# Total-RD/pymgrid

Measured on AMD Instinct MI355X. Metric: microgrid env-steps/sec, higher is better.
Workload: dtype f64

## Files before the change

pymgrid_amd/_lib.py:

```python
import ctypes as C
import json
import os
import re
import subprocess
import sys

_PKG = os.path.dirname(os.path.abspath(__file__))
_ROOT = os.path.dirname(_PKG)
LIB_PATH = os.environ.get("MGX_LIB") or os.path.join(_PKG, "libmgx.so")
SOURCES = [os.path.join(_PKG, "csrc", f) for f in ("mgx_abi.hip", "mgx_fused.hip", "mgx_kernels.hpp", "mgx_core.hpp", "mgx_episodes.hip",
                                                      "mgx_step_episodes.hip")] + \
          [os.path.join(_ROOT, "include", "mgx.h")]
FUSED_PARTS = 6
EPISODE_PARTS = 2
STEP_EPISODE_PARTS = 2

HIPCC_FLAGS = ["--offload-arch=gfx950", "-O3", "-std=c++17", "-ffp-contract=off", "-fno-fast-math", "-fPIC"]

MGX_OK, MGX_ERR_INVALID, MGX_ERR_UNSUPPORTED, MGX_ERR_RANGE, MGX_ERR_DEVICE = range(5)
V_GENSET_RANGE, V_BATTERY_LIMIT, V_GRID_LIMIT, V_GENSET_GOAL, V_GENSET_NEGATIVE, V_NEGATIVE_LIMIT = 1, 2, 4, 8, 16, 32
V_EXPAND_CONSUME, V_EXPAND_PRODUCE, V_EXPAND_SIGN = 64, 128, 256
V_EXPAND = V_EXPAND_CONSUME | V_EXPAND_PRODUCE | V_EXPAND_SIGN
V_ASSERTS = V_GENSET_GOAL | V_GENSET_NEGATIVE | V_NEGATIVE_LIMIT | V_EXPAND
ABI_VERSION = 9
ABI_MINOR = 3
TUNABLES = ("win_threads", "win_group", "win_pairs", "win_min_lds", "prefetch_pool", "multi_generic", "multi_small_own",
            "grid_major_copy", "fleet_byvalue", "launch_threads", "multi_static", "fleet_episodes")
MAX_INSTANCES = 8


class MgxError(RuntimeError):
    def __init__(self, code, message):
        super().__init__(f"[mgx error {code}] {message}")
        self.code = code


c_double_p = C.POINTER(C.c_double)
c_u32_p = C.POINTER(C.c_uint32)
c_u8_p = C.POINTER(C.c_uint8)
c_i32_p = C.POINTER(C.c_int32)


class Layout(C.Structure):
    _fields_ = [(n, C.c_int32) for n in (
# ... 321 lines not shown
```

pymgrid_amd/csrc/mgx_core.hpp:

```cpp
#pragma once

#include <hip/hip_runtime.h>
#include <stdint.h>

#include "../../include/mgx.h"

namespace mgx {

enum : int { F_GENSET = 1, F_BATTERY = 2, F_GRID = 4, F_GRID_FIRST = 8 };

enum LogCol : int {
    LC_REWARD = 0, LC_FIXED_PROVIDED, LC_FIXED_ABSORBED, LC_CTRL_PROVIDED, LC_CTRL_ABSORBED,
    LC_OVERALL_PROVIDED, LC_OVERALL_ABSORBED,
    LC_LOAD_MET, LC_RENEWABLE_USED, LC_CURTAILMENT, LC_LOSS_LOAD, LC_OVERGENERATION, LC_UNBALANCED_REWARD,
    LC_COMMON_END,
    LC_GENSET_N = 4, LC_BATTERY_N = 5, LC_GRID_N = 4
};

struct KArgs {
    mgx_columns c;
    int32_t N, T, H, final_step;
    int32_t obs_dim, log_dim;
    int32_t n_load, n_pv;
    int32_t n_genset, n_battery, n_grid;
    int32_t obs_f32;
    int32_t act_f32;
    int32_t obs_state_only;
    int32_t done_bits;
    int32_t obs_colpitch;
    int32_t col_load, col_pv, col_gen, col_bat, col_grid;
    int32_t shaper;
    int32_t noise_increase;
    uint64_t noise_seed;
    int32_t *t_dev;
    int32_t g0, g1;
    const int32_t *grid_final;
    int32_t row_mask;
    int32_t *ep_off, *ep_final;
// ... 40 lines not shown
        if (prev == gridDim.x - 1) {
            const int32_t t = __hip_atomic_load(&a.t_dev[0], __ATOMIC_RELAXED, __HIP_MEMORY_SCOPE_AGENT);
            __hip_atomic_store(&a.t_dev[2], 0, __ATOMIC_RELAXED, __HIP_MEMORY_SCOPE_AGENT);
            __hip_atomic_store(&a.t_dev[0], t + k, __ATOMIC_RELEASE, __HIP_MEMORY_SCOPE_AGENT);
        }
    }
}

__device__ __forceinline__ int32_t resolve_t_obs(const KArgs &a, int32_t t) { return a.t_dev ? a.t_dev[0] + t : t; }

__device__ __forceinline__ int32_t resolve_k(const KArgs &a, int32_t t0, int32_t K)
{
    if (a.t_dev && t0 + K > a.T) { a.t_dev[1] = 1; return a.T - t0; }
    return K;
}

struct Params {
    double bat_cmin, bat_cmax, bat_C, bat_D, bat_eta, bat_cost;
    double gen_rmin, gen_rmax, gen_cost, gen_co2, gen_cco2;
    uint32_t gen_times;
    double grid_imp, grid_exp, grid_cco2;
    double ll_cost, og_cost;
};

struct State {
    double charge, soc;
    uint32_t status;
};

struct Derived {
    double bat_lo, bat_sp;
    double gen_sp;
    double grid_lo, grid_sp;
};

struct Inputs {
    double a_goal, a_gen, a_bat, a_grid;
    double load, pv;
    double g_pimp, g_pexp, g_co2, g_stat;
};

struct Outputs {
    double reward;
    double fixed_provided, fixed_absorbed, ctrl_provided, ctrl_absorbed, overall_provided, overall_absorbed;
    double load_met, renewable_used, curtailment, loss_load, overgeneration, unbalanced_reward;
    double genset_production, genset_co2, genset_reward;
    double discharge_amount, charge_amount, battery_reward, soc_pre, charge_pre;
    double grid_import, grid_export, grid_co2, grid_reward;
    uint32_t violations;
};

__device__ __forceinline__ double space_spread(double lo, double hi)
{
    double s = hi - lo;
    return s == 0.0 ? 1.0 : s;
}
__device__ __forceinline__ double space_denorm(double lo, double hi, double v) { return lo + space_spread(lo, hi) * v; }
__device__ __forceinline__ double space_norm(double lo, double hi, double v) { return (v - lo) / space_spread(lo, hi); }

__device__ __forceinline__ double py_min(double a, double b)
{
    double r;
    asm("v_min_f64 %0, %1, %2" : "=v"(r) : "v"(a), "v"(b));
    return r;
}
__device__ __forceinline__ double py_max(double a, double b)
{
    double r;
    asm("v_max_f64 %0, %1, %2" : "=v"(r) : "v"(a), "v"(b));
    return r;
}
__device__ __forceinline__ double py_clip(double x, double lo, double hi) { return py_min(py_max(x, lo), hi); }

template <int F>
__device__ __forceinline__ void derive(const Params &p, Derived &d)
{
    if constexpr (F & F_BATTERY) {
        d.bat_lo = -p.bat_D / p.bat_eta;
        d.bat_sp = space_spread(d.bat_lo, p.bat_C * p.bat_eta);
    }
    if constexpr (F & F_GENSET) d.gen_sp = space_spread(0.0, p.gen_rmax);
    if constexpr (F & F_GRID) {
        d.grid_lo = -1 * p.grid_exp;
        d.grid_sp = space_spread(d.grid_lo, p.grid_imp);
    }
}

constexpr int PP = MGX_PROFILE_PITCH;

__host__ __device__ __forceinline__ bool factorised(const mgx_columns &c) { return c.base_load != nullptr; }

struct GridFactors {
    double lr, pr;
    uint32_t lp, pp, cp, pat;
};

template <int F>
__device__ __forceinline__ void load_factors(const mgx_columns &c, int64_t i, GridFactors &f)
{
    f.lr = c.load_ratio[i]; f.pr = c.pv_ratio[i];
    f.lp = c.load_profile[i]; f.pp = c.pv_profile[i];
    f.cp = 0u; f.pat = 0u;
    if constexpr (F & F_GRID) { f.cp = c.co2_profile[i]; f.pat = c.tariff[i]; }
}

__device__ __forceinline__ int64_t base_index(int32_t pm, int64_t row, uint32_t p)
{
    return pm ? (int64_t)p * pm + row : row * PP + p;
}

__device__ __forceinline__ double fact_load(double base, double ratio) { return -1.0 * fabs(base * ratio); }
__device__ __forceinline__ double fact_pv(double base, double ratio) { return fabs(base * ratio); }

__device__ __forceinline__ double tariff_price(int32_t pattern, int32_t row)
{
    const int32_t h = row % 24;
    if (pattern == 1) return (h >= 12 && h < 18) ? 0.59 : ((h < 8 || h >= 21) ? 0.22 : 0.29);
// ... 163 lines not shown
            }
            if (gs != cur) { if (gs == 0) down -= 1; else up -= 1; }
        }
    }
    return (uint32_t)cur | ((uint32_t)gs << 8) | ((uint32_t)(up & 0xff) << 16) | ((uint32_t)(down & 0xff) << 24);
}

__device__ __forceinline__ int genset_next_status(uint32_t st, int goal)
{
    const int cur = st & 0xff, up = (st >> 16) & 0xff, down = st >> 24;
    if (goal) return (cur || up == 0) ? 1 : 0;
    return (!cur || down == 0) ? 0 : 1;
}

template <int F>
__device__ __forceinline__ bool genset_wave_is_instant(const Params &p, const State &s)
{
    if constexpr (F & F_GENSET)
        return __all((p.gen_times == 0u) && (s.status == 0u || s.status == 0x0101u)) != 0;
    return false;
}

__device__ __forceinline__ double battery_max_production(const Params &p, double charge)
{
    const double b = charge - p.bat_cmin;
    return py_min(p.bat_D, b) * p.bat_eta;
}
__device__ __forceinline__ double battery_max_consumption(const Params &p, double charge)
{
    const double b = p.bat_cmax - charge;
    return py_min(p.bat_C, b) / p.bat_eta;
}

template <int F, bool HAVE_Q = false>
__device__ __forceinline__ void step_core(const Params &p, const Derived &d, State &s, const Inputs &in, bool normalized,
                                          bool want_soc, bool gen_instant, Outputs &o, double bat_q = 0.0)
{
    double prov = 0.0, absb = 0.0, reward = 0.0;
    uint32_t viol = 0u;

    const double L = -1 * in.load;
    o.load_met = L;
    absb += L; reward += 0.0;
    o.fixed_provided = prov; o.fixed_absorbed = absb;

    if constexpr (F & F_GENSET) {
        if (gen_instant) {
            const uint32_t g = in.a_goal > 0.5 ? 1u : 0u;
            s.status = g | (g << 8);
        } else {
            s.status = genset_update_status(s.status, p.gen_times, in.a_goal);
        }
        const double x = normalized ? 0.0 + d.gen_sp * in.a_gen : in.a_gen;
        const double cur = (double)(s.status & 0xff);
        const double mx = cur * p.gen_rmax, mn = cur * p.gen_rmin;
        const double e = py_clip(x, mn, mx);
        viol |= ((x > mx) || (x < mn) ? 1u : 0u) | (!(in.a_goal >= 0.0 && in.a_goal <= 1.0) ? 8u : 0u) | (x < 0.0 ? 16u : 0u);
        const double co2 = p.gen_co2 * e;
        const double cost = p.gen_cost * e + p.gen_cco2 * co2;
        o.genset_production = e; o.genset_co2 = co2; o.genset_reward = -1.0 * cost;
        prov += e; reward += o.genset_reward;
    }

    auto step_battery = [&]() __attribute__((always_inline)) {
        const double x = normalized ? d.bat_lo + d.bat_sp * in.a_bat : in.a_bat;
        o.soc_pre = s.soc; o.charge_pre = s.charge;
        const bool sink = x < 0;
        const double room = p.bat_cmax - s.charge;
        const double num_sink = py_min(p.bat_C, room);
        const double mp = battery_max_production(p, s.charge);
        const double e_src = py_clip(x, 0.0, mp);
        const double num = sink ? num_sink : -1.0 * e_src;
        double q;
        if constexpr (HAVE_Q) q = bat_q; else q = num / p.bat_eta;
        const double ex = -1.0 * x;
        const double e_sink = py_min(ex, q);
        const double e = sink ? e_sink : e_src;
        viol |= (sink ? (ex > q) : (x > mp)) ? 2u : 0u;
        viol |= !((sink ? e_sink : e_src) >= 0) ? 32u : 0u;
        const double internal = sink ? e * p.bat_eta : ((num < 0) ? q : num * p.bat_eta);
        o.charge_amount = sink ? e : 0.0;
        o.discharge_amount = sink ? 0.0 : e;
        absb += o.charge_amount; prov += o.discharge_amount;
        s.charge = py_max(s.charge + internal, p.bat_cmin);
        if (want_soc) s.soc = s.charge / p.bat_cmax;
        o.battery_reward = -1.0 * (fabs(internal) * p.bat_cost);
        reward += o.battery_reward;
    };
    auto step_grid = [&]() __attribute__((always_inline)) {
        const double x = normalized ? d.grid_lo + d.grid_sp * in.a_grid : in.a_grid;
        const bool sink = x < 0;
        const double ex = -1.0 * x, mc = p.grid_exp * in.g_stat;
        const double e_exp = py_min(ex, mc);
        const double mp = p.grid_imp * in.g_stat;
        const double e_imp = py_clip(x, 0.0, mp);
        viol |= (sink ? (ex > mc) : (x > mp)) ? 4u : 0u;
        viol |= !((sink ? e_exp : e_imp) >= 0) ? 32u : 0u;
        const double co2 = sink ? 0.0 : e_imp * in.g_co2;
        const double cco2 = -1.0 * p.grid_cco2 * co2;
        o.grid_export = sink ? e_exp : 0.0;
        o.grid_import = sink ? 0.0 : e_imp;
        o.grid_co2 = co2;
        o.grid_reward = sink ? in.g_pexp * e_exp + cco2 : -1 * in.g_pimp * e_imp + cco2;
        absb += o.grid_export; prov += o.grid_import;
        reward += o.grid_reward;
    };
    if constexpr ((F & F_GRID_FIRST) != 0) {
        if constexpr (F & F_GRID) step_grid();
        if constexpr (F & F_BATTERY) step_battery();
    } else {
        if constexpr (F & F_BATTERY) step_battery();
        if constexpr (F & F_GRID) step_grid();
    }

    const double difference = prov - absb;
    o.ctrl_provided = prov - o.fixed_provided;
    o.ctrl_absorbed = absb - o.fixed_absorbed;

    const bool excess = difference > 0;
    const double need = -difference;
    const double used = excess ? 0.0 : py_min(need, in.pv);
    o.renewable_used = used; o.curtailment = in.pv - used;
    const double loss = excess ? 0.0 : need - used;
    const double over = excess ? difference : 0.0;
    o.loss_load = loss; o.overgeneration = over;
    o.unbalanced_reward = -1.0 * (excess ? p.og_cost * over : p.ll_cost * loss);
    prov += used; reward += 0.0;
    prov += loss;
    absb += over;
    reward += o.unbalanced_reward;
    o.overall_provided = prov; o.overall_absorbed = absb;
    o.reward = reward;
    o.violations = viol;
}

struct PLWords {
    uint32_t w[12];
    int32_t n_actions;
};

__device__ __forceinline__ uint32_t pl_select(const PLWords &tab, int32_t id)
{
    uint32_t w = tab.w[0];
#pragma unroll
    for (int j = 1; j < 12; j++) w = (id == j && j < tab.n_actions) ? tab.w[j] : w;
    return w;
}

__device__ __forceinline__ bool pl_isclose0(double rem)
{
    return fabs(rem - 0.0) <= 1e-4 + 1e-5 * fabs(0.0);
}

__device__ __forceinline__ double pl_energy(double rem, double mn, double mx, double mc, bool is_sink)
{
    const double produce = py_clip(rem, mn, mx);
    const double consume = is_sink ? py_max(rem, -1.0 * mc) : 0.0;
    return pl_isclose0(rem) ? 0.0 : ((rem > 0) ? produce : consume);
}

template <int F, bool CHECK = false>
__device__ __forceinline__ void populate_core(const Params &p, const State &s, uint32_t word, Inputs &in, double &bat_q,
                                              double total_load, double renewable, bool gen_instant = false,
                                              uint32_t *xviol = nullptr, bool check_sign = true)
{
    const double rem0 = total_load - renewable;
    double g_mx[2] = {0.0, 0.0}, g_mn[2] = {0.0, 0.0};
    if constexpr (F & F_GENSET) {
#pragma unroll
        for (int act = 0; act < 2; act++) {
            const double ns = gen_instant ? (double)act : (double)genset_next_status(s.status, act);
            g_mx[act] = ns * p.gen_rmax; g_mn[act] = ns * p.gen_rmin;
        }
    }
    double r_mx = 0.0, r_mc = 0.0;
    if constexpr (F & F_GRID) { r_mx = p.grid_imp * in.g_stat; r_mc = p.grid_exp * in.g_stat; }

    constexpr int NSLOT = ((F & F_GENSET) != 0) + ((F & F_BATTERY) != 0) + ((F & F_GRID) != 0);
    constexpr int NS = NSLOT > 0 ? NSLOT : 1;
    uint32_t el[NS];
#pragma unroll
    for (int k = 0; k < NS; k++) el[k] = (k < NSLOT) ? (word >> (4 * k)) & 0xfu : 0u;
    auto cheap = [&](int mod, int act, double rem) -> double {
        double e = 0.0;
        if constexpr ((F & F_GENSET) && (F & F_GRID))
            e = (mod == 0) ? pl_energy(rem, g_mn[act], g_mx[act], 0.0, false) : pl_energy(rem, 0.0, r_mx, r_mc, true);
        else if constexpr (F & F_GENSET)
            e = pl_energy(rem, g_mn[act], g_mx[act], 0.0, false);
        else if constexpr (F & F_GRID)
            e = pl_energy(rem, 0.0, r_mx, r_mc, true);
        return e;
    };

    double remB = rem0;
    if constexpr (F & F_BATTERY) {
        double rem = rem0;
        bool seen = false;
#pragma unroll
        for (int k = 0; k < NSLOT - 1; k++) {
            const bool valid = (el[k] & 8u) != 0;
            const int mod = el[k] & 3u, act = (el[k] >> 2) & 1u;
            const bool isB = valid && mod == 1;
            seen = seen || isB;
            rem -= (valid && !seen) ? cheap(mod, act, rem) : 0.0;
            remB = seen ? remB : rem;
        }
    }
    double eB = 0.0;
    bat_q = 0.0;
    if constexpr (F & F_BATTERY) {
        const bool close = pl_isclose0(remB);
        const bool produce = !close && remB > 0;
        const double mp = battery_max_production(p, s.charge);
        const double room = p.bat_cmax - s.charge;
        const double num_sink = py_min(p.bat_C, room);
        const double e_src = py_clip(remB, 0.0, mp);
        const double num = (close || produce) ? -1.0 * (produce ? e_src : 0.0) : num_sink;
        const double q = num / p.bat_eta;
        const double e_snk = py_max(remB, -1.0 * q);
        eB = close ? 0.0 : (produce ? e_src : e_snk);
        bat_q = q;
    }
    double rem = rem0, c_goal = 0.0, c_gen = 0.0, c_grid = 0.0;
    uint32_t xv = 0u;
    if constexpr (CHECK) xv = (check_sign && !(total_load >= 0 && renewable >= 0)) ? 256u : 0u;
#pragma unroll
    for (int k = 0; k < NSLOT; k++) {
        const bool valid = (el[k] & 8u) != 0;
        const int mod = el[k] & 3u, act = (el[k] >> 2) & 1u;
        const double e = (mod == 1) ? eB : cheap(mod, act, rem);
        if constexpr (CHECK) {
            const bool close = pl_isclose0(rem), produce = !close && rem > 0, consume = !close && !produce;
            const double mc = (mod == 1) ? bat_q : r_mc;
            uint32_t bad = (produce && !(e >= 0)) ? 128u : 0u;
            bad = (consume && !(rem <= 0.0)) ? 256u : bad;
            bad = (consume && rem <= 0.0 && mod != 0 && !(mc >= 0)) ? 64u : bad;
            xv = (xv == 0u && valid) ? bad : xv;
        }
        const bool isG = valid && mod == 0, isR = valid && mod == 2;
        c_goal = isG ? (double)act : c_goal;
        c_gen = isG ? e : c_gen;
        c_grid = isR ? e : c_grid;
        rem -= valid ? e : 0.0;
    }
    in.a_goal = c_goal; in.a_gen = c_gen; in.a_bat = eB; in.a_grid = c_grid;
    if constexpr (CHECK) { if (xviol) *xviol = xv; }
}

template <int F>
__device__ __forceinline__ double shaped_reward(int32_t shaper, const Outputs &o)
{
// ... 1054 lines not shown
```

pymgrid_amd/csrc/mgx_episodes.hip:

```cpp
#include "mgx_kernels.hpp"

#ifndef MGX_EPISODE_PART
#error "compile with -DMGX_EPISODE_PART=<0..MGX_EPISODE_PARTS-1>"
#endif

#if MGX_EPISODE_PART == 0
#define MGX_PART_FLAGS(X) X(0) X(1) X(2) X(3) X(4) X(5)
#elif MGX_EPISODE_PART == 1
#define MGX_PART_FLAGS(X) X(6) X(7) X(14) X(15)
#else
#error "MGX_EPISODE_PART out of range"
#endif

#define MGX_CAT2(a, b) a##b
#define MGX_CAT(a, b) MGX_CAT2(a, b)

namespace mgx {

struct EpisodeSlot {
    double load, pv, g_pimp, g_pexp, g_co2, g_stat;
    uint64_t outage;
};

template <int F, int U, bool PER_STEP, int SRC>
__global__ __launch_bounds__(BLOCK_K) void rollout_episodes_kernel(const KArgs a, const PLWords tab, const uint8_t *__restrict__ ids,
                                                                   int32_t t0, int32_t K, const FusedOut out,
                                                                   const mgx_episode_stats es, int32_t gpb,
                                                                   const KArgs *__restrict__ a_dev)
{
    static_assert(U <= 8, "the id ring is one 64-bit register");
    constexpr bool FACT = SRC == EP_SRC_FACT;
    const int64_t i = (int64_t)blockIdx.x * gpb + threadIdx.x;
    __shared__ uint32_t word_of_id[PER_STEP ? BLOCK_K : 1];
    if constexpr (PER_STEP) {
        static_assert(BLOCK_K == 256, "one thread per id byte");
        word_of_id[threadIdx.x] = pl_select(tab, (int32_t)threadIdx.x);
        __syncthreads();
    }
    if ((int32_t)threadIdx.x >= gpb || i >= a.N) return;
    const int64_t N = a.N;
    const int32_t pm = a.pm_pitch;
    const uint32_t i32 = (uint32_t)i;
    Params p; State s; Derived d;
    load_state<F>(a.c, i, false, s);
    load_params<F>(a.c, i, p);
    derive<F>(p, d);
    const bool gen_instant = genset_wave_is_instant<F>(p, s);
    const bool want_soc = out.soc_trace != nullptr;
    const bool ar_on = a.ar_mode != 0;
    int32_t off = a.ep_off[i], fin = a.ep_final[i];
    uint32_t word = PER_STEP ? 0u : pl_select(tab, ids[i]);
    GridFactors f;
    f.lr = 0.0; f.pr = 0.0; f.lp = 0u; f.pp = 0u; f.cp = 0u; f.pat = 0u;
    if constexpr (FACT) load_factors<F>(a.c, i, f);
    double run = es.ret_running ? es.ret_running[i] : 0.0;
    double sum = es.ret_sum ? es.ret_sum[i] : 0.0;
    double last = es.ret_last ? es.ret_last[i] : 0.0;
    int32_t eps = es.episodes ? es.episodes[i] : 0;

    auto fetch = [&](EpisodeSlot &r, int32_t t) __attribute__((always_inline)) {
        const int64_t row = episode_row(a, t, off);
        if constexpr (SRC == EP_SRC_FACT) {
            r.load = a.c.base_load[(int64_t)f.lp * pm + row];
            r.pv = a.c.base_pv[(int64_t)f.pp * pm + row];
            if constexpr (F & F_GRID) {
                r.g_co2 = a.c.base_co2[(int64_t)f.cp * pm + row];
                r.outage = 0;
                if (a.c.outage_bits) r.outage = a.c.outage_bits[(row >> 6) * N + i];
            }
        } else if constexpr (SRC == EP_SRC_GRID_MAJOR) {
            constexpr int C = (F & F_GRID) ? 6 : 2;
            const double2 *q = reinterpret_cast<const double2 *>(a.c.load_ts + (i * pm + row) * C);
            const double2 v0 = q[0];
            r.load = v0.x; r.pv = v0.y;
            if constexpr (F & F_GRID) {
                const double2 v1 = q[1], v2 = q[2];
                r.g_pimp = v1.x; r.g_pexp = v1.y; r.g_co2 = v2.x; r.g_stat = v2.y;
            }
        } else {
// ... 22 lines not shown
        }
    };

    {
        const bool GI = gen_instant;
        EpisodeSlot ring[U];
        uint64_t idq = 0;
#pragma unroll
        for (int u = 0; u < U; u++)
            if (u < K) {
                fetch(ring[u], t0 + u);
                if constexpr (PER_STEP) idq |= (uint64_t)(ids + (int64_t)u * N)[i32] << (8 * u);
            }
        uint32_t word_next = 0u;
        if constexpr (PER_STEP) word_next = word_of_id[idq & 0xffu];
        int64_t o64 = i;
#pragma nounroll
        for (int32_t k = 0; k < K; k++) {
            const int32_t t = t0 + k;
            Inputs in;
            widen_slot(ring[0], t, in);
#pragma unroll
            for (int u = 0; u + 1 < U; u++) ring[u] = ring[u + 1];
            if constexpr (PER_STEP) {
                word = word_next;
                idq >>= 8;
                word_next = word_of_id[idq & 0xffu];
                if (k + U < K) idq |= (uint64_t)(ids + (int64_t)(k + U) * N)[i32] << (8 * (U - 1));
            } else {
                asm volatile("" : "+v"(word));
            }
            double bat_q;
            uint32_t xv = 0u;
            populate_core<F, false>(p, s, word, in, bat_q, 0.0 + -1 * in.load, in.pv, GI, &xv);
            Outputs o;
            step_core<F, true>(p, d, s, in, false, want_soc, GI, o, bat_q);
            const double r = shaped_reward<F>(a.shaper, o);
            const bool dn = t >= fin - 1;
            if (out.reward) out.reward[o64] = r;
            if (out.done) out.done[o64] = (uint8_t)dn;
            if constexpr (F & F_BATTERY) { if (out.soc_trace) out.soc_trace[o64] = s.soc; }
            if constexpr (F & F_GENSET) { if (out.status_trace) out.status_trace[o64] = s.status; }
            o64 += N;
            run += r;
            if (t == fin - 1) { last = run; sum += run; eps += 1; run = 0.0; }
            if (ar_on && dn) {
                off = episode_auto_restart(*a_dev, i, t, off, true);
                fin = a_dev->ep_final[i];
#pragma unroll
                for (int v = 0; v < U; v++)
                    if (k + 1 + v < K) fetch(ring[v], t + 1 + v);
            } else if (k + U < K) {
                fetch(ring[U - 1], t + U);
            }
        }
    }
    if constexpr (F & F_BATTERY) { if (!want_soc) s.soc = s.charge / p.bat_cmax; }
    store_state<F>(a_dev->c, i, s);
    if (es.ret_running) es.ret_running[i] = run;
    if (es.ret_sum) es.ret_sum[i] = sum;
    if (es.ret_last) es.ret_last[i] = last;
    if (es.episodes) es.episodes[i] = eps;
}

template <int F>
static void rollout_episodes_dispatch(const EpisodeLaunch &L)
{
#define MGX_EPISODES(PS, SRC) rollout_episodes_kernel<F, (F & F_GRID) ? 4 : MGX_RING_ROLLOUT, PS, SRC><<<L.blocks, BLOCK_K, 0, L.stream>>>( \
        *L.k, *L.tab, L.ids, L.t, L.K, L.out, L.stats, L.gpb, L.k_dev)
// ... 24 lines not shown
```

pymgrid_amd/csrc/mgx_kernels.hpp:

```cpp
#pragma once
#include "mgx_core.hpp"

#include <type_traits>

namespace mgx {

#ifndef MGX_BLOCK
#define MGX_BLOCK 128
#endif
constexpr int BLOCK = MGX_BLOCK;
#ifndef MGX_RING
#define MGX_RING 8
#endif
#ifndef MGX_RING_RICH
#define MGX_RING_RICH 16
#endif
#ifndef MGX_BLOCK_K
#define MGX_BLOCK_K 256
#endif
constexpr int BLOCK_K = MGX_BLOCK_K;
#ifndef MGX_RING_ROLLOUT
#define MGX_RING_ROLLOUT 8
#endif

// ... 304 lines not shown
};

template <int F, typename AT>
__device__ __forceinline__ void load_actions_at(const AT *__restrict__ row, uint32_t i32, RawActions<AT> &r)
{
    constexpr int A = 2 * ((F & F_GENSET) != 0) + ((F & F_BATTERY) != 0) + ((F & F_GRID) != 0);
    const AT *a = row + i32 * (uint32_t)A;
    int k = 0;
#if MGX_ACT_NT
    if constexpr (F & F_GENSET) { r.a_goal = __builtin_nontemporal_load(a + k); r.a_gen = __builtin_nontemporal_load(a + k + 1); k += 2; }
    if constexpr (F & F_BATTERY) { r.a_bat = __builtin_nontemporal_load(a + k); k += 1; }
    if constexpr (F & F_GRID) { r.a_grid = __builtin_nontemporal_load(a + k); k += 1; }
#else
    if constexpr (F & F_GENSET) { r.a_goal = a[k]; r.a_gen = a[k + 1]; k += 2; }
    if constexpr (F & F_BATTERY) { r.a_bat = a[k]; k += 1; }
    if constexpr (F & F_GRID) { r.a_grid = a[k]; k += 1; }
#endif
}

__device__ __forceinline__ void store_done(const KArgs &a, uint8_t *__restrict__ done, int64_t off, int64_t i, int32_t k, bool dn)
{
    if (a.done_bits) {
        const unsigned long long b = __ballot(dn);
        const int lane = threadIdx.x & 63;
        if ((lane & 15) == 0) {
            const int64_t W = ((int64_t)a.N + 15) >> 4;
            reinterpret_cast<uint16_t *>(done)[(int64_t)k * W + (i >> 4)] = (uint16_t)(b >> (lane & 48));
        }
    } else {
        done[off] = (uint8_t)dn;
    }
}

template <int F, int U, typename AT, bool RICH, bool FACT>
__global__ __launch_bounds__(BLOCK_K) void step_k_kernel(const KArgs a, const AT *__restrict__ actions, int32_t t0,
                                                         int32_t K, int normalized, const FusedOut out_rt, int32_t gpb)
{
    FusedOut out = out_rt;
    if constexpr (!RICH) { out.log = nullptr; out.status_trace = nullptr; }
    const int32_t K_launch = K;
    t0 = resolve_t(a, t0);
    K = resolve_k(a, t0, K);
    const int64_t i = (int64_t)a.g0 + (int64_t)blockIdx.x * gpb + threadIdx.x;
    const bool active = (int32_t)threadIdx.x < gpb && i < a.g1;
    if constexpr (!FACT) { if (!active) return; }
    const int64_t N = a.N;
    constexpr int A_DIM = 2 * ((F & F_GENSET) != 0) + ((F & F_BATTERY) != 0) + ((F & F_GRID) != 0);
    Params p; State s; Derived d;
    const bool norm = normalized != 0;
    const bool want_soc = (out.soc_trace != nullptr) || (out.log != nullptr);
    bool gen_instant = false;
    int32_t k_done = 0;
    if (active) {
        load_state<F>(a.c, i, out.log != nullptr, s);
        load_params<F>(a.c, i, p);
        derive<F>(p, d);
        gen_instant = genset_wave_is_instant<F>(p, s);
        k_done = (a.grid_final ? a.grid_final[i] : a.final_step) - 1 - t0;
    }
    double ret = 0.0;

    const bool hot = !RICH && out.reward != nullptr && out.done == nullptr && (!(F & F_BATTERY) || out.soc_trace != nullptr) &&
                     a.shaper == MGX_SHAPER_NONE;
    const uint32_t i32 = (uint32_t)i;
    auto consume = [&](auto gi_tag, auto hot_tag, const Inputs &in, int32_t k, int64_t off) __attribute__((always_inline)) {
        constexpr bool GI = decltype(gi_tag)::value, HOT = decltype(hot_tag)::value;
        Outputs o;
        step_core<F>(p, d, s, in, norm, HOT ? (F & F_BATTERY) != 0 : want_soc, GI, o);
        if constexpr (HOT) {
            const double r = o.reward;
#if MGX_HOT_NT
            __builtin_nontemporal_store(r, (out.reward + (int64_t)k * N) + i32);
            if constexpr (F & F_BATTERY) __builtin_nontemporal_store(s.soc, (out.soc_trace + (int64_t)k * N) + i32);
#else
            (out.reward + (int64_t)k * N)[i32] = r;
            if constexpr (F & F_BATTERY) (out.soc_trace + (int64_t)k * N)[i32] = s.soc;
#endif
            ret += r;
            return;
        }
        const double r = shaped_reward<F>(a.shaper, o);
        {
#if MGX_OUT_NT
            if (out.reward) __builtin_nontemporal_store(r, out.reward + off);
            if (out.done) store_done(a, out.done, off, i, k, k >= k_done);
            if constexpr (F & F_BATTERY) { if (out.soc_trace) __builtin_nontemporal_store(s.soc, out.soc_trace + off); }
            if constexpr (F & F_GENSET) { if (out.status_trace) __builtin_nontemporal_store(s.status, out.status_trace + off); }
#else
            if (out.reward) out.reward[off] = r;
            if (out.done) store_done(a, out.done, off, i, k, k >= k_done);
            if constexpr (F & F_BATTERY) { if (out.soc_trace) out.soc_trace[off] = s.soc; }
            if constexpr (F & F_GENSET) { if (out.status_trace) out.status_trace[off] = s.status; }
#endif
            if (out.log) store_log<F>(out.log + (off - i) * a.log_dim + i, N, o, s.status);
        }
        ret += r;
    };
    auto specialised = [&](auto fn) __attribute__((always_inline)) {
        if constexpr ((F & F_GENSET) != 0) {
            if (gen_instant) { if (hot) fn(std::true_type{}, std::true_type{}); else fn(std::true_type{}, std::false_type{}); }
            else { if (hot) fn(std::false_type{}, std::true_type{}); else fn(std::false_type{}, std::false_type{}); }
        } else {
            if (hot) fn(std::false_type{}, std::true_type{}); else fn(std::false_type{}, std::false_type{});
        }
    };

    if constexpr (FACT) {
        __shared__ double base_lds[((F & F_GRID) ? 3 : 2) * FACT_ROWS * PP];
        static_assert(FACT_ROWS % U == 0, "ring slots are addressed by k % U across LDS chunks");
        GridFactors f;
        f.lr = 0.0; f.pr = 0.0; f.lp = 0u; f.pp = 0u; f.cp = 0u; f.pat = 0u;
        OutageWords ow;
        ow.cur = 0; ow.nxt = 0; ow.wi = 0;
        RawActions<AT> ring[U];
        if (active) {
            load_factors<F>(a.c, i, f);
            if constexpr (F & F_GRID) outage_init(a.c, N, i, a.T, t0, ow);
#pragma unroll
            for (int u = 0; u < U; u++)
                if (u < K) load_actions_at<F>(actions + (int64_t)u * N * A_DIM, i32, ring[u]);
        }
        int64_t off = i;
        auto run_chunk = [&](auto gi_tag, auto hot_tag, int32_t kb, int32_t n) __attribute__((always_inline)) {
            BaseVals nb = read_base_row<F>(base_lds, 0, f);
            for (int32_t k0 = kb; k0 < kb + n; k0 += U) {
#pragma unroll
                for (int u = 0; u < U; u++) {
                    const int32_t k = k0 + u;
                    if (k < kb + n) {
                        const RawActions<AT> ra = ring[u];
                        if (k + U < K) load_actions_at<F>(actions + (int64_t)(k + U) * N * A_DIM, i32, ring[u]);
                        Inputs in;
                        if constexpr (F & F_GENSET) { in.a_goal = (double)ra.a_goal; in.a_gen = (double)ra.a_gen; }
                        if constexpr (F & F_BATTERY) in.a_bat = (double)ra.a_bat;
                        in.load = fact_load(nb.load, f.lr);
                        in.pv = fact_pv(nb.pv, f.pr);
                        if constexpr (F & F_GRID) {
                            in.a_grid = (double)ra.a_grid;
                            in.g_pimp = tariff_price((int32_t)f.pat, t0 + k); in.g_pexp = 0.0;
                            in.g_co2 = nb.co2;
                            in.g_stat = outage_status(a.c, N, i, a.T, t0 + k, k == 0, ow);
                        }
                        const int32_t rn = (k + 1 - kb < n) ? k + 1 - kb : n - 1;
                        nb = read_base_row<F>(base_lds, rn, f);
                        consume(gi_tag, hot_tag, in, k, off);
                        off += N;
                    }
                }
            }
        };
        for (int32_t kb = 0; kb < K; kb += FACT_ROWS) {
            const int32_t n = K - kb < FACT_ROWS ? K - kb : FACT_ROWS;
            __syncthreads();
            stage_base_rows<F>(a.c, (int64_t)t0 + kb, n, base_lds, BLOCK_K);
            __syncthreads();
            if (active) specialised([&](auto gi_tag, auto hot_tag) __attribute__((always_inline)) { run_chunk(gi_tag, hot_tag, kb, n); });
        }
        if (!active) return;
    } else {
        const double *__restrict__ lts = a.c.load_ts + (int64_t)t0 * N;
        const double *__restrict__ pts = a.c.pv_ts + (int64_t)t0 * N;
        const double *__restrict__ gts = (F & F_GRID) ? a.c.grid_ts + (int64_t)t0 * 4 * N : nullptr;
        specialised([&](auto gi_tag, auto hot_tag) __attribute__((always_inline)) {
            RawInputs<AT> ring[U];
#pragma unroll
            for (int u = 0; u < U; u++)
                if (u < K) load_inputs_at<F>(actions, lts, pts, gts, N, i, (int64_t)u * N + i, ring[u]);

            int64_t off = i;
            for (int32_t k0 = 0; k0 < K; k0 += U) {
#pragma unroll
                for (int u = 0; u < U; u++) {
                    const int32_t k = k0 + u;
                    if (k < K) {
                        const Inputs in = widen<F>(ring[u]);
                        if (k + U < K) load_inputs_at<F>(actions, lts, pts, gts, N, i, off + (int64_t)U * N, ring[u]);
                        consume(gi_tag, hot_tag, in, k, off);
                        off += N;
                    }
                }
            }
        });
    }
    if constexpr (F & F_BATTERY) { if (!want_soc) s.soc = s.charge / p.bat_cmax; }
    store_state<F>(a.c, i, s);
    if (out.ret_acc) out.ret_acc[i] += ret;
    advance_counter_in_kernel(a, K_launch);
}

struct FusedLaunch {
    int flags;
    bool act_f32, rich, fact, per_step;
    unsigned blocks;
    hipStream_t stream;
    const KArgs *k;
    const void *actions;
    const PLWords *tab;
    const uint8_t *ids;
    int32_t t, K;
    int normalized;
    FusedOut out;
    int32_t gpb;
};
constexpr int MGX_FUSED_PARTS = 6;
struct MultiStaticLaunch {
    int flags, ng, nb, nr, nl, np;
    unsigned blocks;
    hipStream_t stream;
    const KArgs *k;
    const void *actions;
    int32_t t, K;
    int normalized;
// ... 828 lines not shown
        MGX_FLEET_V_STEP(0, EPV) MGX_FLEET_V_STEP(1, EPV) MGX_FLEET_V_STEP(2, EPV) MGX_FLEET_V_STEP(3, EPV) MGX_FLEET_V_STEP(4, EPV)   \
        MGX_FLEET_V_STEP(5, EPV) MGX_FLEET_V_STEP(6, EPV) MGX_FLEET_V_STEP(7, EPV) MGX_FLEET_V_STEP(14, EPV)                          \
        default: { step_body<15, EPV>(B.k, B.actions, hd.t, normalized, B.reward, B.done, B.obs, B.log, i); } break;                  \
    }

template <bool EP>
static __global__ __launch_bounds__(BLOCK) void fleet_step_kernel_v(const FleetArgsV fa)
{
    MGX_FLEET_V_HEAD
    MGX_FLEET_V_SWITCHES(EP)
}

template <int F, int U, bool PER_STEP, bool RICH, bool FACT>
__global__ __launch_bounds__(BLOCK_K) void rollout_kernel(const KArgs a, const PLWords tab, const uint8_t *__restrict__ ids,
                                                          int32_t t0, int32_t K, const FusedOut out_rt, int32_t gpb)
{
    FusedOut out = out_rt;
    if constexpr (!RICH) { out.log = nullptr; out.status_trace = nullptr; }
    const int32_t K_launch = K;
    t0 = resolve_t(a, t0);
    K = resolve_k(a, t0, K);
    const int64_t i = (int64_t)a.g0 + (int64_t)blockIdx.x * gpb + threadIdx.x;
    const bool active = (int32_t)threadIdx.x < gpb && i < a.g1;
    if constexpr (!FACT) { if (!active) return; }
    const int64_t N = a.N;
    Params p; State s; Derived d;
    const bool want_soc = (out.soc_trace != nullptr) || (out.log != nullptr);
    bool gen_instant = false;
    int32_t k_done = 0;
    uint32_t word = 0u;
    if (active) {
        load_state<F>(a.c, i, out.log != nullptr, s);
        load_params<F>(a.c, i, p);
        derive<F>(p, d);
        gen_instant = genset_wave_is_instant<F>(p, s);
        k_done = (a.grid_final ? a.grid_final[i] : a.final_step) - 1 - t0;
        word = PER_STEP ? 0u : pl_select(tab, ids[i]);
    }
    double ret = 0.0;

    const bool hot = !RICH && out.reward != nullptr && out.done == nullptr && (!(F & F_BATTERY) || out.soc_trace != nullptr) &&
                     a.shaper == MGX_SHAPER_NONE;
    const uint32_t i32 = (uint32_t)i;
    auto consume = [&](auto gi_tag, auto hot_tag, Inputs &in, int32_t k, int64_t off) __attribute__((always_inline)) {
        constexpr bool GI = decltype(gi_tag)::value, HOT = decltype(hot_tag)::value;
        double bat_q;
        uint32_t xv = 0u;
        populate_core<F, RICH>(p, s, word, in, bat_q, 0.0 + -1 * in.load, in.pv, GI, &xv);
        Outputs o;
        step_core<F, true>(p, d, s, in, false, HOT ? (F & F_BATTERY) != 0 : want_soc, GI, o, bat_q);
        if constexpr (RICH) o.violations |= xv;
        if constexpr (HOT) {
            const double r = o.reward;
            (out.reward + (int64_t)k * N)[i32] = r;
            if constexpr (F & F_BATTERY) (out.soc_trace + (int64_t)k * N)[i32] = s.soc;
            ret += r;
            return;
        }
        const double r = shaped_reward<F>(a.shaper, o);
        if (out.reward) out.reward[off] = r;
        if (out.done) store_done(a, out.done, off, i, k, k >= k_done);
        if constexpr (F & F_BATTERY) { if (out.soc_trace) out.soc_trace[off] = s.soc; }
        if constexpr (F & F_GENSET) { if (out.status_trace) out.status_trace[off] = s.status; }
        if (out.log) store_log<F>(out.log + (off - i) * a.log_dim + i, N, o, s.status);
        ret += r;
    };
    auto specialised = [&](auto fn) __attribute__((always_inline)) {
        if constexpr ((F & F_GENSET) != 0) {
            if (gen_instant) { if (hot) fn(std::true_type{}, std::true_type{}); else fn(std::true_type{}, std::false_type{}); }
            else { if (hot) fn(std::false_type{}, std::true_type{}); else fn(std::false_type{}, std::false_type{}); }
        } else {
            if (hot) fn(std::false_type{}, std::true_type{}); else fn(std::false_type{}, std::false_type{});
        }
    };
    if constexpr (FACT) {
        __shared__ double base_lds[((F & F_GRID) ? 3 : 2) * FACT_ROWS * PP];
        static_assert(FACT_ROWS % U == 0, "ring slots are addressed by k % U across LDS chunks");
        GridFactors f;
        f.lr = 0.0; f.pr = 0.0; f.lp = 0u; f.pp = 0u; f.cp = 0u; f.pat = 0u;
        OutageWords ow;
        ow.cur = 0; ow.nxt = 0; ow.wi = 0;
        static_assert(U <= 8, "the id ring is one 64-bit register");
        uint64_t idq = 0;
// ... 1176 lines not shown
```

pymgrid_amd/csrc/mgx_step_episodes.hip:

```cpp
#include "mgx_kernels.hpp"

#ifndef MGX_STEP_EPISODE_PART
#error "compile with -DMGX_STEP_EPISODE_PART=<0..MGX_STEP_EPISODE_PARTS-1>"
#endif

#if MGX_STEP_EPISODE_PART == 0
#define MGX_PART_FLAGS(X) X(0) X(1) X(2) X(3) X(4) X(5)
#elif MGX_STEP_EPISODE_PART == 1
#define MGX_PART_FLAGS(X) X(6) X(7) X(14) X(15)
#else
#error "MGX_STEP_EPISODE_PART out of range"
#endif

#ifndef MGX_RING_STEP_EPISODES
#define MGX_RING_STEP_EPISODES 4
#endif

#define MGX_CAT2(a, b) a##b
#define MGX_CAT(a, b) MGX_CAT2(a, b)

namespace mgx {

struct SeriesSlot {
    double load, pv, g_pimp, g_pexp, g_co2, g_stat;
    uint64_t outage;
};

template <int F, int U, int UA, typename AT, int SRC>
__global__ __launch_bounds__(BLOCK_K) void step_k_episodes_kernel(const KArgs a, const AT *__restrict__ actions, int32_t t0, int32_t K,
                                                                  int normalized, const FusedOut out, const mgx_episode_stats es,
                                                                  int32_t gpb, const KArgs *__restrict__ a_dev)
{
    constexpr bool FACT = SRC == EP_SRC_FACT;
    constexpr int A_DIM = 2 * ((F & F_GENSET) != 0) + ((F & F_BATTERY) != 0) + ((F & F_GRID) != 0);
    const int64_t i = (int64_t)blockIdx.x * gpb + threadIdx.x;
    if ((int32_t)threadIdx.x >= gpb || i >= a.N) return;
    const int64_t N = a.N;
    const int32_t pm = a.pm_pitch;
    const uint32_t i32 = (uint32_t)i;
    Params p; State s; Derived d;
    load_state<F>(a.c, i, false, s);
    load_params<F>(a.c, i, p);
    derive<F>(p, d);
    const bool gen_instant = genset_wave_is_instant<F>(p, s);
    const bool norm = normalized != 0;
    const bool want_soc = out.soc_trace != nullptr;
    const bool ar_on = a.ar_mode != 0;
    int32_t off = a.ep_off[i], fin = a.ep_final[i];
    GridFactors f;
    f.lr = 0.0; f.pr = 0.0; f.lp = 0u; f.pp = 0u; f.cp = 0u; f.pat = 0u;
    if constexpr (FACT) load_factors<F>(a.c, i, f);
    double run = es.ret_running ? es.ret_running[i] : 0.0;
    double sum = es.ret_sum ? es.ret_sum[i] : 0.0;
    double last = es.ret_last ? es.ret_last[i] : 0.0;
    int32_t eps = es.episodes ? es.episodes[i] : 0;

    auto fetch = [&](SeriesSlot &r, int32_t t) __attribute__((always_inline)) {
        const int64_t row = episode_row(a, t, off);
        if constexpr (SRC == EP_SRC_FACT) {
            r.load = a.c.base_load[(int64_t)f.lp * pm + row];
            r.pv = a.c.base_pv[(int64_t)f.pp * pm + row];
            if constexpr (F & F_GRID) {
                r.g_co2 = a.c.base_co2[(int64_t)f.cp * pm + row];
                r.outage = 0;
                if (a.c.outage_bits) r.outage = a.c.outage_bits[(row >> 6) * N + i];
            }
        } else if constexpr (SRC == EP_SRC_GRID_MAJOR) {
            constexpr int C = (F & F_GRID) ? 6 : 2;
            const double2 *q = reinterpret_cast<const double2 *>(a.c.load_ts + (i * pm + row) * C);
            const double2 v0 = q[0];
            r.load = v0.x; r.pv = v0.y;
            if constexpr (F & F_GRID) {
                const double2 v1 = q[1], v2 = q[2];
                r.g_pimp = v1.x; r.g_pexp = v1.y; r.g_co2 = v2.x; r.g_stat = v2.y;
            }
        } else {
            r.load = a.c.load_ts[row * N + i];
            r.pv = a.c.pv_ts[row * N + i];
// ... 16 lines not shown
            }
        } else {
            in.load = r.load; in.pv = r.pv;
            if constexpr (F & F_GRID) { in.g_pimp = r.g_pimp; in.g_pexp = r.g_pexp; in.g_co2 = r.g_co2; in.g_stat = r.g_stat; }
        }
    };

    {
        const bool GI = gen_instant;
        SeriesSlot ring[U];
        RawActions<AT> act[UA];
#pragma unroll
        for (int u = 0; u < U; u++)
            if (u < K) fetch(ring[u], t0 + u);
        const AT *arow = actions;
#pragma unroll
        for (int u = 0; u < UA; u++)
            if (u < K) { load_actions_at<F>(arow, i32, act[u]); arow += N * A_DIM; }
        int64_t o64 = i;
#pragma nounroll
        for (int32_t k = 0; k < K; k++) {
            const int32_t t = t0 + k;
            Inputs in;
            widen_slot(ring[0], t, in);
            if constexpr (F & F_GENSET) { in.a_goal = (double)act[0].a_goal; in.a_gen = (double)act[0].a_gen; }
            if constexpr (F & F_BATTERY) in.a_bat = (double)act[0].a_bat;
            if constexpr (F & F_GRID) in.a_grid = (double)act[0].a_grid;
#pragma unroll
            for (int u = 0; u + 1 < U; u++) ring[u] = ring[u + 1];
#pragma unroll
            for (int u = 0; u + 1 < UA; u++) act[u] = act[u + 1];
            if (k + UA < K) { load_actions_at<F>(arow, i32, act[UA - 1]); arow += N * A_DIM; }
            Outputs o;
            step_core<F>(p, d, s, in, norm, want_soc, GI, o);
            const double r = shaped_reward<F>(a.shaper, o);
            const bool dn = t >= fin - 1;
            if (out.reward) out.reward[o64] = r;
            if (out.done) out.done[o64] = (uint8_t)dn;
            if constexpr (F & F_BATTERY) { if (out.soc_trace) out.soc_trace[o64] = s.soc; }
            if constexpr (F & F_GENSET) { if (out.status_trace) out.status_trace[o64] = s.status; }
            o64 += N;
            run += r;
            if (t == fin - 1) { last = run; sum += run; eps += 1; run = 0.0; }
            if (ar_on && dn) {
                off = episode_auto_restart(*a_dev, i, t, off, true);
                fin = a_dev->ep_final[i];
#pragma unroll
                for (int v = 0; v < U; v++)
                    if (k + 1 + v < K) fetch(ring[v], t + 1 + v);
            } else if (k + U < K) {
                fetch(ring[U - 1], t + U);
            }
        }
    }
    if constexpr (F & F_BATTERY) { if (!want_soc) s.soc = s.charge / p.bat_cmax; }
    store_state<F>(a_dev->c, i, s);
    if (es.ret_running) es.ret_running[i] = run;
    if (es.ret_sum) es.ret_sum[i] = sum;
    if (es.ret_last) es.ret_last[i] = last;
    if (es.episodes) es.episodes[i] = eps;
}

template <int F, typename AT>
static void step_k_episodes_dispatch(const StepEpisodeLaunch &L)
{
#define MGX_STEP_EPISODES(SRC) step_k_episodes_kernel<F, (F & F_GRID) ? 4 : MGX_RING_ROLLOUT, MGX_RING_STEP_EPISODES, AT, SRC><<<L.blocks, BLOCK_K, 0, L.stream>>>( \
        *L.k, (const AT *)L.actions, L.t, L.K, L.normalized, L.out, L.stats, L.gpb, L.k_dev)
// ... 18 lines not shown
```

Before: 134.6 billion.

## Replace per-step f64 divisions with reciprocal-refined exact division and peel steady-state loops

Precomputes reciprocals of battery efficiency and capacity once per env and replaces the per-step f64 divisions with a multiply plus two FMA Newton refinements. A guarded fallback to true division handles extreme magnitudes, so results stay bit-exact. Normalization is folded into the derived affine constants (identity when not normalized), which removes a per-step branch. Select operands are computed eagerly for branchless selection. The step loops are peeled into a steady-state part with no bounds checks. The trade-off is extra FMAs and more register pressure, and a traffic-only debug path is added behind a macro that is off by default.

```diff
diff --git a/pymgrid_amd/_lib.py b/pymgrid_amd/_lib.py
--- a/pymgrid_amd/_lib.py
+++ b/pymgrid_amd/_lib.py
@@ -9,7 +9,7 @@
 _ROOT = os.path.dirname(_PKG)
 LIB_PATH = os.environ.get("MGX_LIB") or os.path.join(_PKG, "libmgx.so")
 SOURCES = [os.path.join(_PKG, "csrc", f) for f in ("mgx_abi.hip", "mgx_fused.hip", "mgx_kernels.hpp", "mgx_core.hpp", "mgx_episodes.hip",
-                                                      "mgx_step_episodes.hip")] + \
+                                                      "mgx_step_episodes.hip", "mgx_exactdiv.hpp")] + \
           [os.path.join(_ROOT, "include", "mgx.h")]
 FUSED_PARTS = 6
 EPISODE_PARTS = 2
diff --git a/pymgrid_amd/csrc/mgx_core.hpp b/pymgrid_amd/csrc/mgx_core.hpp
--- a/pymgrid_amd/csrc/mgx_core.hpp
+++ b/pymgrid_amd/csrc/mgx_core.hpp
@@ -4,6 +4,7 @@
 #include <stdint.h>
 
 #include "../../include/mgx.h"
+#include "mgx_exactdiv.hpp"
 
 namespace mgx {
 
@@ -110,6 +111,7 @@
     double bat_lo, bat_sp;
     double gen_sp;
     double grid_lo, grid_sp;
+    ExactDiv div_eta, div_cmax;
 };
 
 struct Inputs {
@@ -161,6 +163,21 @@
     if constexpr (F & F_GRID) {
         d.grid_lo = -1 * p.grid_exp;
         d.grid_sp = space_spread(d.grid_lo, p.grid_imp);
+    }
+}
+
+template <int F>
+__device__ __forceinline__ void derive_fused(const Params &p, bool normalized, Derived &d)
+{
+    derive<F>(p, d);
+    if (!normalized) {
+        if constexpr (F & F_BATTERY) { d.bat_lo = 0.0; d.bat_sp = 1.0; }
+        if constexpr (F & F_GENSET) d.gen_sp = 1.0;
+        if constexpr (F & F_GRID) { d.grid_lo = 0.0; d.grid_sp = 1.0; }
+    }
+    if constexpr (F & F_BATTERY) {
+        d.div_eta = exactdiv_setup(p.bat_eta);
+        d.div_cmax = exactdiv_setup(p.bat_cmax);
     }
 }
 
@@ -390,7 +407,7 @@
     return py_min(p.bat_C, b) / p.bat_eta;
 }
 
-template <int F, bool HAVE_Q = false>
+template <int F, bool HAVE_Q = false, bool FUSED = false>
 __device__ __forceinline__ void step_core(const Params &p, const Derived &d, State &s, const Inputs &in, bool normalized,
                                           bool want_soc, bool gen_instant, Outputs &o, double bat_q = 0.0)
 {
@@ -430,18 +447,27 @@
         const double e_src = py_clip(x, 0.0, mp);
         const double num = sink ? num_sink : -1.0 * e_src;
         double q;
-        if constexpr (HAVE_Q) q = bat_q; else q = num / p.bat_eta;
+        if constexpr (HAVE_Q) q = bat_q;
+        else if constexpr (FUSED) q = exactdiv(d.div_eta, num);
+        else q = num / p.bat_eta;
         const double ex = -1.0 * x;
         const double e_sink = py_min(ex, q);
         const double e = sink ? e_sink : e_src;
         viol |= (sink ? (ex > q) : (x > mp)) ? 2u : 0u;
         viol |= !((sink ? e_sink : e_src) >= 0) ? 32u : 0u;
-        const double internal = sink ? e * p.bat_eta : ((num < 0) ? q : num * p.bat_eta);
+        double internal;
+        if constexpr (FUSED) {
+            const double i_sink = e_sink * p.bat_eta, i_src = num * p.bat_eta;
+            internal = sink ? i_sink : ((num < 0) ? q : i_src);
+        } else {
+            internal = sink ? e * p.bat_eta : ((num < 0) ? q : num * p.bat_eta);
+        }
         o.charge_amount = sink ? e : 0.0;
         o.discharge_amount = sink ? 0.0 : e;
         absb += o.charge_amount; prov += o.discharge_amount;
         s.charge = py_max(s.charge + internal, p.bat_cmin);
-        if (want_soc) s.soc = s.charge / p.bat_cmax;
+        if constexpr (FUSED) { if (want_soc) s.soc = exactdiv(d.div_cmax, s.charge); }
+        else { if (want_soc) s.soc = s.charge / p.bat_cmax; }
         o.battery_reward = -1.0 * (fabs(internal) * p.bat_cost);
         reward += o.battery_reward;
     };
@@ -477,12 +503,19 @@
 
     const bool excess = difference > 0;
     const double need = -difference;
-    const double used = excess ? 0.0 : py_min(need, in.pv);
+    double used;
+    if constexpr (FUSED) { const double m = py_min(need, in.pv); used = excess ? 0.0 : m; }
+    else used = excess ? 0.0 : py_min(need, in.pv);
     o.renewable_used = used; o.curtailment = in.pv - used;
     const double loss = excess ? 0.0 : need - used;
     const double over = excess ? difference : 0.0;
     o.loss_load = loss; o.overgeneration = over;
-    o.unbalanced_reward = -1.0 * (excess ? p.og_cost * over : p.ll_cost * loss);
+    if constexpr (FUSED) {
+        const double c_over = p.og_cost * over, c_loss = p.ll_cost * loss;
+        o.unbalanced_reward = -1.0 * (excess ? c_over : c_loss);
+    } else {
+        o.unbalanced_reward = -1.0 * (excess ? p.og_cost * over : p.ll_cost * loss);
+    }
     prov += used; reward += 0.0;
     prov += loss;
     absb += over;
@@ -520,7 +553,7 @@
 template <int F, bool CHECK = false>
 __device__ __forceinline__ void populate_core(const Params &p, const State &s, uint32_t word, Inputs &in, double &bat_q,
                                               double total_load, double renewable, bool gen_instant = false,
-                                              uint32_t *xviol = nullptr, bool check_sign = true)
+                                              uint32_t *xviol = nullptr, bool check_sign = true, const Derived *dd = nullptr)
 {
     const double rem0 = total_load - renewable;
     double g_mx[2] = {0.0, 0.0}, g_mn[2] = {0.0, 0.0};
@@ -574,7 +607,7 @@
         const double num_sink = py_min(p.bat_C, room);
         const double e_src = py_clip(remB, 0.0, mp);
         const double num = (close || produce) ? -1.0 * (produce ? e_src : 0.0) : num_sink;
-        const double q = num / p.bat_eta;
+        const double q = dd ? exactdiv(dd->div_eta, num) : num / p.bat_eta;
         const double e_snk = py_max(remB, -1.0 * q);
         eB = close ? 0.0 : (produce ? e_src : e_snk);
         bat_q = q;
diff --git a/pymgrid_amd/csrc/mgx_episodes.hip b/pymgrid_amd/csrc/mgx_episodes.hip
--- a/pymgrid_amd/csrc/mgx_episodes.hip
+++ b/pymgrid_amd/csrc/mgx_episodes.hip
@@ -44,7 +44,7 @@
     Params p; State s; Derived d;
     load_state<F>(a.c, i, false, s);
     load_params<F>(a.c, i, p);
-    derive<F>(p, d);
+    derive_fused<F>(p, false, d);
     const bool gen_instant = genset_wave_is_instant<F>(p, s);
     const bool want_soc = out.soc_trace != nullptr;
     const bool ar_on = a.ar_mode != 0;
@@ -133,9 +133,9 @@
             }
             double bat_q;
             uint32_t xv = 0u;
-            populate_core<F, false>(p, s, word, in, bat_q, 0.0 + -1 * in.load, in.pv, GI, &xv);
+            populate_core<F, false>(p, s, word, in, bat_q, 0.0 + -1 * in.load, in.pv, GI, &xv, true, &d);
             Outputs o;
-            step_core<F, true>(p, d, s, in, false, want_soc, GI, o, bat_q);
+            step_core<F, true, true>(p, d, s, in, false, want_soc, GI, o, bat_q);
             const double r = shaped_reward<F>(a.shaper, o);
             const bool dn = t >= fin - 1;
             if (out.reward) out.reward[o64] = r;
diff --git a/pymgrid_amd/csrc/mgx_exactdiv.hpp b/pymgrid_amd/csrc/mgx_exactdiv.hpp
--- /dev/null
+++ b/pymgrid_amd/csrc/mgx_exactdiv.hpp
@@ -0,0 +1,37 @@
+#pragma once
+#include <math.h>
+
+#if defined(__HIPCC__) || defined(__CUDACC__)
+#define MGX_EXACTDIV_FN __host__ __device__ __forceinline__
+#else
+#define MGX_EXACTDIV_FN inline
+#endif
+
+namespace mgx {
+
+struct ExactDiv {
+    double d;
+    double y;
+};
+
+MGX_EXACTDIV_FN ExactDiv exactdiv_setup(double d)
+{
+    ExactDiv e;
+    e.d = d;
+    const double ad = fabs(d);
+    const bool fast = ad >= 0x1p-100 && ad <= 0x1p100;
+    e.y = fast ? 1.0 / d : NAN;
+    return e;
+}
+
+MGX_EXACTDIV_FN double exactdiv(const ExactDiv &e, double n)
+{
+    double q = n * e.y;
+    q = fma(fma(-e.d, q, n), e.y, q);
+    q = fma(fma(-e.d, q, n), e.y, q);
+    const bool ok = ((fabs(n) >= 0x1p-800) | (n == 0.0)) & (fabs(q) <= 0x1.fffffffffffffp1023);
+    if (__builtin_expect(!ok, 0)) q = n / e.d;
+    return q;
+}
+
+}
diff --git a/pymgrid_amd/csrc/mgx_kernels.hpp b/pymgrid_amd/csrc/mgx_kernels.hpp
--- a/pymgrid_amd/csrc/mgx_kernels.hpp
+++ b/pymgrid_amd/csrc/mgx_kernels.hpp
@@ -360,6 +360,20 @@
     }
 }
 
+#ifndef MGX_TRAFFIC_ONLY
+#define MGX_TRAFFIC_ONLY 0
+#endif
+template <int F>
+__device__ __forceinline__ void traffic_only_core(const Inputs &in, State &s, Outputs &o)
+{
+    o = Outputs{};
+    double v = in.load + in.pv;
+    if constexpr (F & F_GENSET) v += in.a_goal + in.a_gen;
+    if constexpr (F & F_BATTERY) { v += in.a_bat; s.soc = v + s.charge; }
+    if constexpr (F & F_GRID) v += in.a_grid + in.g_pimp + in.g_pexp + in.g_co2 + in.g_stat;
+    o.reward = v;
+}
+
 template <int F, int U, typename AT, bool RICH, bool FACT>
 __global__ __launch_bounds__(BLOCK_K) void step_k_kernel(const KArgs a, const AT *__restrict__ actions, int32_t t0,
                                                          int32_t K, int normalized, const FusedOut out_rt, int32_t gpb)
@@ -382,7 +396,7 @@
     if (active) {
         load_state<F>(a.c, i, out.log != nullptr, s);
         load_params<F>(a.c, i, p);
-        derive<F>(p, d);
+        derive_fused<F>(p, norm, d);
         gen_instant = genset_wave_is_instant<F>(p, s);
         k_done = (a.grid_final ? a.grid_final[i] : a.final_step) - 1 - t0;
     }
@@ -394,7 +408,11 @@
     auto consume = [&](auto gi_tag, auto hot_tag, const Inputs &in, int32_t k, int64_t off) __attribute__((always_inline)) {
         constexpr bool GI = decltype(gi_tag)::value, HOT = decltype(hot_tag)::value;
         Outputs o;
-        step_core<F>(p, d, s, in, norm, HOT ? (F & F_BATTERY) != 0 : want_soc, GI, o);
+#if MGX_TRAFFIC_ONLY
+        traffic_only_core<F>(in, s, o);
+#else
+        step_core<F, false, true>(p, d, s, in, true, HOT ? (F & F_BATTERY) != 0 : want_soc, GI, o);
+#endif
         if constexpr (HOT) {
             const double r = o.reward;
 #if MGX_HOT_NT
@@ -451,29 +469,35 @@
         int64_t off = i;
         auto run_chunk = [&](auto gi_tag, auto hot_tag, int32_t kb, int32_t n) __attribute__((always_inline)) {
             BaseVals nb = read_base_row<F>(base_lds, 0, f);
-            for (int32_t k0 = kb; k0 < kb + n; k0 += U) {
+            auto one = [&](auto steady_tag, int u, int32_t k) __attribute__((always_inline)) {
+                const RawActions<AT> ra = ring[u];
+                if (decltype(steady_tag)::value || k + U < K) load_actions_at<F>(actions + (int64_t)(k + U) * N * A_DIM, i32, ring[u]);
+                Inputs in;
+                if constexpr (F & F_GENSET) { in.a_goal = (double)ra.a_goal; in.a_gen = (double)ra.a_gen; }
+                if constexpr (F & F_BATTERY) in.a_bat = (double)ra.a_bat;
+                in.load = fact_load(nb.load, f.lr);
+                in.pv = fact_pv(nb.pv, f.pr);
+                if constexpr (F & F_GRID) {
+                    in.a_grid = (double)ra.a_grid;
+                    in.g_pimp = tariff_price((int32_t)f.pat, t0 + k); in.g_pexp = 0.0;
+                    in.g_co2 = nb.co2;
+                    in.g_stat = outage_status(a.c, N, i, a.T, t0 + k, k == 0, ow);
+                }
+                const int32_t rn = (k + 1 - kb < n) ? k + 1 - kb : n - 1;
+                nb = read_base_row<F>(base_lds, rn, f);
+                consume(gi_tag, hot_tag, in, k, off);
+                off += N;
+            };
+            int32_t k0 = kb;
+            for (; k0 + U <= kb + n && k0 + 2 * U <= K; k0 += U) {
+#pragma unroll
+                for (int u = 0; u < U; u++) one(std::true_type{}, u, k0 + u);
+            }
+            for (; k0 < kb + n; k0 += U) {
 #pragma unroll
                 for (int u = 0; u < U; u++) {
                     const int32_t k = k0 + u;
-                    if (k < kb + n) {
-                        const RawActions<AT> ra = ring[u];
-                        if (k + U < K) load_actions_at<F>(actions + (int64_t)(k + U) * N * A_DIM, i32, ring[u]);
-                        Inputs in;
-                        if constexpr (F & F_GENSET) { in.a_goal = (double)ra.a_goal; in.a_gen = (double)ra.a_gen; }
-                        if constexpr (F & F_BATTERY) in.a_bat = (double)ra.a_bat;
-                        in.load = fact_load(nb.load, f.lr);
-                        in.pv = fact_pv(nb.pv, f.pr);
-                        if constexpr (F & F_GRID) {
-                            in.a_grid = (double)ra.a_grid;
-                            in.g_pimp = tariff_price((int32_t)f.pat, t0 + k); in.g_pexp = 0.0;
-                            in.g_co2 = nb.co2;
-                            in.g_stat = outage_status(a.c, N, i, a.T, t0 + k, k == 0, ow);
-                        }
-                        const int32_t rn = (k + 1 - kb < n) ? k + 1 - kb : n - 1;
-                        nb = read_base_row<F>(base_lds, rn, f);
-                        consume(gi_tag, hot_tag, in, k, off);
-                        off += N;
-                    }
+                    if (k < kb + n) one(std::false_type{}, u, k);
                 }
             }
         };
@@ -496,16 +520,24 @@
                 if (u < K) load_inputs_at<F>(actions, lts, pts, gts, N, i, (int64_t)u * N + i, ring[u]);
 
             int64_t off = i;
-            for (int32_t k0 = 0; k0 < K; k0 += U) {
+            auto one = [&](auto steady_tag, int u, int32_t k) __attribute__((always_inline)) {
+                const Inputs in = widen<F>(ring[u]);
+                if (decltype(steady_tag)::value || k + U < K) load_inputs_at<F>(actions, lts, pts, gts, N, i, off + (int64_t)U * N, ring[u]);
+                consume(gi_tag, hot_tag, in, k, off);
+                off += N;
+            };
+            int32_t k0 = 0;
+            if constexpr (!RICH) {
+                for (; k0 + 2 * U <= K; k0 += U) {
+#pragma unroll
+                    for (int u = 0; u < U; u++) one(std::true_type{}, u, k0 + u);
+                }
+            }
+            for (; k0 < K; k0 += U) {
 #pragma unroll
                 for (int u = 0; u < U; u++) {
                     const int32_t k = k0 + u;
-                    if (k < K) {
-                        const Inputs in = widen<F>(ring[u]);
-                        if (k + U < K) load_inputs_at<F>(actions, lts, pts, gts, N, i, off + (int64_t)U * N, ring[u]);
-                        consume(gi_tag, hot_tag, in, k, off);
-                        off += N;
-                    }
+                    if (k < K) one(std::false_type{}, u, k);
                 }
             }
         });
@@ -1400,7 +1432,7 @@
     if (active) {
         load_state<F>(a.c, i, out.log != nullptr, s);
         load_params<F>(a.c, i, p);
-        derive<F>(p, d);
+        derive_fused<F>(p, false, d);
         gen_instant = genset_wave_is_instant<F>(p, s);
         k_done = (a.grid_final ? a.grid_final[i] : a.final_step) - 1 - t0;
         word = PER_STEP ? 0u : pl_select(tab, ids[i]);
@@ -1414,9 +1446,9 @@
         constexpr bool GI = decltype(gi_tag)::value, HOT = decltype(hot_tag)::value;
         double bat_q;
         uint32_t xv = 0u;
-        populate_core<F, RICH>(p, s, word, in, bat_q, 0.0 + -1 * in.load, in.pv, GI, &xv);
+        populate_core<F, RICH>(p, s, word, in, bat_q, 0.0 + -1 * in.load, in.pv, GI, &xv, true, &d);
         Outputs o;
-        step_core<F, true>(p, d, s, in, false, HOT ? (F & F_BATTERY) != 0 : want_soc, GI, o, bat_q);
+        step_core<F, true, true>(p, d, s, in, false, HOT ? (F & F_BATTERY) != 0 : want_soc, GI, o, bat_q);
         if constexpr (RICH) o.violations |= xv;
         if constexpr (HOT) {
             const double r = o.reward;
diff --git a/pymgrid_amd/csrc/mgx_step_episodes.hip b/pymgrid_amd/csrc/mgx_step_episodes.hip
--- a/pymgrid_amd/csrc/mgx_step_episodes.hip
+++ b/pymgrid_amd/csrc/mgx_step_episodes.hip
@@ -41,9 +41,9 @@
     Params p; State s; Derived d;
     load_state<F>(a.c, i, false, s);
     load_params<F>(a.c, i, p);
-    derive<F>(p, d);
+    const bool norm = normalized != 0;
+    derive_fused<F>(p, norm, d);
     const bool gen_instant = genset_wave_is_instant<F>(p, s);
-    const bool norm = normalized != 0;
     const bool want_soc = out.soc_trace != nullptr;
     const bool ar_on = a.ar_mode != 0;
     int32_t off = a.ep_off[i], fin = a.ep_final[i];
@@ -126,7 +126,7 @@
             for (int u = 0; u + 1 < UA; u++) act[u] = act[u + 1];
             if (k + UA < K) { load_actions_at<F>(arow, i32, act[UA - 1]); arow += N * A_DIM; }
             Outputs o;
-            step_core<F>(p, d, s, in, norm, want_soc, GI, o);
+            step_core<F, false, true>(p, d, s, in, true, want_soc, GI, o);
             const double r = shaped_reward<F>(a.shaper, o);
             const bool dn = t >= fin - 1;
             if (out.reward) out.reward[o64] = r;
```

Result: slower. 117.2 billion (-12.9%).
